# bdaiinstitute/judo

Hardware: AMD Instinct MI355X
Metric: rollouts/sec + plan-step ms, leap_cube MPPI 65536xH64 (higher is better)
Workload: dtype f32

## Files before the change

### include/judo_amd.h

```cpp
#ifndef JUDO_AMD_H
#define JUDO_AMD_H

#include <stddef.h>
#include <stdint.h>

#ifdef __cplusplus
extern "C" {
#endif

typedef struct jh_model jh_model;

enum jh_status {
  JH_OK = 0,
  JH_ERR_INVALID = -1,
  JH_ERR_HIP = -2,
  JH_ERR_UNSUPPORTED = -3,
  JH_ERR_BLOB = -4
};

enum jh_task_kind { JH_TASK_CARTPOLE = 0, JH_TASK_CYLINDER_PUSH = 1, JH_TASK_LEAP_CUBE = 2, JH_TASK_FR3_PICK = 3 };
enum jh_spline_kind { JH_SPLINE_ZERO = 0, JH_SPLINE_LINEAR = 1, JH_SPLINE_CUBIC = 3 };

#define JH_MAX_TASK_PARAMS 32
#define JH_MAX_KNOT_DIM 512
#define JH_MAX_ELITES 32

const char* jh_last_error(void);
int jh_version(void);

int jh_model_create(const void* blob, size_t nbytes, int device, jh_model** out);
void jh_model_destroy(jh_model* m);
int jh_model_dims(const jh_model* m, int* dims );

int jh_model_stats(jh_model* m, int* out , int reset);


int jh_model_set_self_collision(jh_model* m, int on);

int jh_model_set_contact_capacity(jh_model* m, int contacts);

int jh_model_build(const jh_model* m, int* out );

int jh_model_trace_layout(const jh_model* m, int* out );
int jh_trace_gather(const float* rec_in , int k, int stride_in, int n_offset, int n_local, const float* trace , int row_floats,
                    int colmajor, float* rec_out , void* stream);

int jh_model_limits(const jh_model* m, int* out );
int jh_model_max_fused_knots(const jh_model* m, int H);
int jh_model_one_launch_max_knots(const jh_model* m, int H);
int jh_model_set_plan_step_launches(jh_model* m, int launches);

int jh_upload_async(void* dst_device, const void* src_host, size_t nbytes, void* stream);
int jh_download_wait(void* dst_host, const void* src_device, size_t nbytes, void* stream);
int jh_download_begin(void* dst_host, const void* src_device, size_t nbytes, void* stream);
int jh_download_end(void);

int jh_rollout_cost(const jh_model* m, const float* x0, const float* nominal, const float* noise, int ldn, const float* sigma,
                    const float* W, const float* ctrl_lo_hi, const float* task_params, int phase, int N, int n_offset, int H, int K,
                    float* costs, float* knots_out, void* stream);
int jh_rollout_cost_traced(const jh_model* m, const float* x0, const float* nominal, const float* noise, int ldn, const float* sigma,
                    const float* W, const float* ctrl_lo_hi, const float* task_params, int phase, int N, int n_offset, int H, int K,
                    float* costs, float* knots_out, float* trace , void* stream);

int jh_rollout_materialize(const jh_model* m, const float* x0, int x0_batched, const float* controls, int N, int H, float* states,
                           float* sensors, void* stream);

int jh_task_reward(const jh_model* m, const float* states, const float* sensors, const float* controls, const float* task_params,
                   int phase, int N, int H, float* rewards, void* stream);

int jh_noise_normal(unsigned long long seed, unsigned int draw, int rows, int n_offset, int n_local, float* out, int ldn, void* stream);

int jh_sample_knots(const float* nominal, const float* noise, int ldn, const float* sigma, const float* ctrl_lo_hi ,
                    int N, int n_offset, int K, int nu, float* knots_nku, void* stream);

int jh_spline_controls(const float* W, const float* knots_nku, const float* nominal, const float* noise, int ldn, const float* sigma,
                       const float* ctrl_lo_hi, int N, int n_offset, int H, int K, int nu, float* controls, void* stream);

int jh_knot_moments(const float* knots_nku, const float* nominal, const float* noise, int ldn, const float* sigma, const float* ctrl_lo_hi,
                    const float* center, int N, int n_offset, int K, int nu, float* out, void* stream);

size_t jh_update_scratch_floats(int N, int K, int nu);
int jh_mppi_partial(const float* costs, const float* knots_nku, const float* nominal, const float* noise, int ldn, const float* sigma,
                    const float* ctrl_lo_hi, int N, int n_offset, int K, int nu, float lambda, float* scratch, float* rec, void* stream);
// ... 56 lines not shown
```

### judo_amd/_lib.py

```python

from __future__ import annotations

import ctypes as C
import os

_HERE = os.path.dirname(os.path.abspath(__file__))
LIB_PATH = os.environ.get("JUDO_AMD_LIB") or os.path.join(_HERE, "libjudo_amd.so")

_lib: C.CDLL | None = None

f32p = C.c_void_p

_SIGNATURES = {
    "jh_last_error": (C.c_char_p, []),
    "jh_version": (C.c_int, []),
    "jh_model_create": (C.c_int, [C.c_void_p, C.c_size_t, C.c_int, C.POINTER(C.c_void_p)]),
    "jh_model_destroy": (None, [C.c_void_p]),
    "jh_model_dims": (C.c_int, [C.c_void_p, C.POINTER(C.c_int)]),
    "jh_model_stats": (C.c_int, [C.c_void_p, C.POINTER(C.c_int), C.c_int]),
    "jh_model_set_kernel": (C.c_int, [C.c_void_p, C.c_int]),
    "jh_model_limits": (C.c_int, [C.c_void_p, C.POINTER(C.c_int)]),
    "jh_register_xcheck": (C.c_int, [C.c_void_p]),
    "jh_model_max_fused_knots": (C.c_int, [C.c_void_p, C.c_int]),
    "jh_model_one_launch_max_knots": (C.c_int, [C.c_void_p, C.c_int]),
    "jh_model_set_plan_step_launches": (C.c_int, [C.c_void_p, C.c_int]),
    "jh_model_set_self_collision": (C.c_int, [C.c_void_p, C.c_int]),
    "jh_model_set_contact_capacity": (C.c_int, [C.c_void_p, C.c_int]),
    "jh_model_build": (C.c_int, [C.c_void_p, C.POINTER(C.c_int)]),
    "jh_model_trace_layout": (C.c_int, [C.c_void_p, C.POINTER(C.c_int)]),
    "jh_trace_gather": (C.c_int, [C.c_void_p, C.c_int, C.c_int, C.c_int, C.c_int, C.c_void_p, C.c_int, C.c_int, C.c_void_p, C.c_void_p]),
    "jh_upload_async": (C.c_int, [C.c_void_p, C.c_void_p, C.c_size_t, C.c_void_p]),
    "jh_download_wait": (C.c_int, [C.c_void_p, C.c_void_p, C.c_size_t, C.c_void_p]),
    "jh_download_begin": (C.c_int, [C.c_void_p, C.c_void_p, C.c_size_t, C.c_void_p]),
    "jh_download_end": (C.c_int, []),
    "jh_rollout_cost": (C.c_int, [C.c_void_p, f32p, f32p, f32p, C.c_int, f32p, f32p, f32p, f32p, C.c_int, C.c_int, C.c_int, C.c_int, C.c_int, f32p, f32p, C.c_void_p]),
    "jh_rollout_cost_traced": (C.c_int, [C.c_void_p, f32p, f32p, f32p, C.c_int, f32p, f32p, f32p, f32p, C.c_int, C.c_int, C.c_int, C.c_int, C.c_int, f32p, f32p, f32p, C.c_void_p]),
    "jh_rollout_materialize": (C.c_int, [C.c_void_p, f32p, C.c_int, f32p, C.c_int, C.c_int, f32p, f32p, C.c_void_p]),
    "jh_task_reward": (C.c_int, [C.c_void_p, f32p, f32p, f32p, f32p, C.c_int, C.c_int, C.c_int, f32p, C.c_void_p]),
    "jh_noise_normal": (C.c_int, [C.c_ulonglong, C.c_uint, C.c_int, C.c_int, C.c_int, f32p, C.c_int, C.c_void_p]),
    "jh_sample_knots": (C.c_int, [f32p, f32p, C.c_int, f32p, f32p, C.c_int, C.c_int, C.c_int, C.c_int, f32p, C.c_void_p]),
    "jh_spline_controls": (C.c_int, [f32p, f32p, f32p, f32p, C.c_int, f32p, f32p, C.c_int, C.c_int, C.c_int, C.c_int, C.c_int, f32p, C.c_void_p]),
    "jh_knot_moments": (C.c_int, [f32p, f32p, f32p, C.c_int, f32p, f32p, f32p, C.c_int, C.c_int, C.c_int, C.c_int, f32p, C.c_void_p]),
    "jh_policy_create": (C.c_int, [C.POINTER(C.c_void_p), C.POINTER(C.c_void_p), C.POINTER(C.c_void_p)]),
    "jh_policy_destroy": (None, [C.c_void_p]),
    "jh_policy_scratch_floats": (C.c_size_t, [C.c_int]),
    "jh_policy_step": (C.c_int, [C.c_void_p, f32p, C.c_int, C.c_int, C.c_int, C.c_int, C.c_int, C.c_int, f32p, f32p, f32p, f32p, C.c_int, C.c_void_p]),
    "jh_tree_create": (C.c_int, [C.c_void_p, C.c_size_t, C.POINTER(C.c_void_p)]),
    "jh_tree_destroy": (None, [C.c_void_p]),
    "jh_tree_stats": (C.c_int, [C.c_void_p, C.POINTER(C.c_int), C.c_int]),
    "jh_tree_dims": (C.c_int, [C.c_void_p, C.POINTER(C.c_int)]),
    "jh_tree_set_self_collision": (C.c_int, [C.c_void_p, C.c_int]),
    "jh_tree_substeps": (C.c_int, [C.c_void_p, f32p, f32p, f32p, C.c_int, C.c_int, f32p, f32p, C.c_void_p]),
    "jh_policy_rollout_scratch_floats": (C.c_size_t, [C.c_int]),
    "jh_policy_rollout": (C.c_int, [C.c_void_p, C.c_void_p, f32p, C.c_int, f32p, f32p, f32p, C.c_int, C.c_int, C.c_int, C.c_int, C.c_double, f32p, f32p, f32p, C.POINTER(C.c_int), C.c_void_p]),
    "jh_update_scratch_floats": (C.c_size_t, [C.c_int, C.c_int, C.c_int]),
    "jh_mppi_partial": (C.c_int, [f32p, f32p, f32p, f32p, C.c_int, f32p, f32p, C.c_int, C.c_int, C.c_int, C.c_int, C.c_float, f32p, f32p, C.c_void_p]),
    "jh_mppi_merge": (C.c_int, [f32p, C.c_int, C.c_int, C.c_int, C.c_float, f32p, C.c_void_p]),
    "jh_topk_partial": (C.c_int, [f32p, f32p, f32p, f32p, C.c_int, f32p, f32p, C.c_int, C.c_int, C.c_int, C.c_int, C.c_int, C.c_int, f32p, f32p, C.c_void_p]),
# ... 62 lines not shown
```

### judo_amd/csrc/jh_api.hip

```cpp
#include <cmath>
#include <cstdlib>
#include <cstring>

#include "jh_internal.h"
#include "jh_update_dev.h"

static thread_local char g_err[512] = "";

void jh_set_error(const char* fmt, ...) {
  va_list ap;
  va_start(ap, fmt);
  vsnprintf(g_err, sizeof(g_err), fmt, ap);
  va_end(ap);
}

extern "C" const char* jh_last_error(void) { return g_err; }
extern "C" int jh_version(void) { return 100; }

static int image_cylinders(const jh_blob_header& h, const float* F, const int* I) {
  constexpr int HEADER = 24, BODY_I = 6, BODY_F = 32, BLOCK_I = 4, DOF_F = 20, ACT_I = 2, ACT_F = 8, GEOM_I = 2, GEOM_F = 20, GF_RBOUND = 15;
  if (h.nint < (uint32_t)HEADER || h.nfloat < (uint32_t)HEADER) return 0;
  const long NM = I[0], NBLK = I[1], nv = I[2], nu = I[4], NG = I[5];
  if (NM < 0 || NBLK < 0 || nv < 0 || nu < 0 || NG < 0) return 0;
  const long oI = HEADER + NM * BODY_I + NBLK * BLOCK_I + nu * ACT_I, oF = HEADER + NM * BODY_F + nv * DOF_F + nu * ACT_F;
// ... 5 lines not shown
    const float r = f[0], L = f[1], rb = f[GF_RBOUND], want = sqrtf(r * r + L * L);
    if (!(r > 0.f) || !(L > 0.f) || f[2] != 0.f) { jh_set_error("model_create: cylinder geom %ld: sizes must be (radius > 0, half length > 0, 0), got (%g, %g, %g)", g, r, L, f[2]); return -1; }
    if (!(fabsf(rb - want) <= 1e-5f * want)) { jh_set_error("model_create: cylinder geom %ld: bounding radius %g is not sqrt(r^2 + L^2) = %g", g, rb, want); return -1; }
    n++;
  }
  return n;
}

extern "C" int jh_model_create(const void* blob, size_t nbytes, int device, jh_model** out) {
  JH_REQUIRE(blob && out, "model_create: null pointer");
  if (nbytes < sizeof(jh_blob_header)) { jh_set_error("model_create: blob too small (%zu bytes)", nbytes); return JH_ERR_BLOB; }
  jh_blob_header h;
  memcpy(&h, blob, sizeof(h));
  if (h.magic != JH_BLOB_MAGIC || h.version != JH_BLOB_VERSION) { jh_set_error("model_create: bad magic/version (%08x, %u)", h.magic, h.version); return JH_ERR_BLOB; }
  size_t need = sizeof(h) + 4 * ((size_t)h.nfloat + h.nint);
  if (nbytes != need) { jh_set_error("model_create: blob size %zu != expected %zu", nbytes, need); return JH_ERR_BLOB; }
  if (h.kind > JH_TASK_FR3_PICK) { jh_set_error("model_create: unknown task kind %u", h.kind); return JH_ERR_BLOB; }
  if (h.kind == JH_TASK_CARTPOLE && h.nfloat < CP_NPARAM) { jh_set_error("model_create: cartpole blob has %u floats, need %d", h.nfloat, CP_NPARAM); return JH_ERR_BLOB; }
  if (h.kind == JH_TASK_CYLINDER_PUSH && h.nfloat < CY_NPARAM) { jh_set_error("model_create: cylinder blob has %u floats, need %d", h.nfloat, CY_NPARAM); return JH_ERR_BLOB; }
  if (h.ntaskparam > JH_MAX_TASK_PARAMS) { jh_set_error("model_create: too many task params"); return JH_ERR_BLOB; }
  int cylinders = 0;
  if (h.kind == JH_TASK_LEAP_CUBE || h.kind == JH_TASK_FR3_PICK) {
    const char* q = (const char*)blob + sizeof(h);
    std::vector<float> F((const float*)q, (const float*)q + h.nfloat);
    std::vector<int> I((const int*)(q + 4 * (size_t)h.nfloat), (const int*)(q + 4 * (size_t)h.nfloat) + h.nint);
    cylinders = image_cylinders(h, F.data(), I.data());
    if (cylinders < 0) return JH_ERR_BLOB;
    if (cylinders > 0 && h.kind != JH_TASK_LEAP_CUBE) { jh_set_error("model_create: %d cylinder geoms, and only the leap kernel has a cylinder build", cylinders); return JH_ERR_BLOB; }
  }
  JH_HIP(hipSetDevice(device));
  jh_model* m = new jh_model();
  m->device = device; m->kind = (int)h.kind; m->nq = h.nq; m->nv = h.nv; m->nu = h.nu; m->ns = h.ns; m->ntaskparam = h.ntaskparam;
  m->nf = h.nfloat; m->ni = h.nint; m->d_f = nullptr; m->d_i = nullptr; m->d_stats = nullptr; m->kernel_gen = (h.kind == JH_TASK_LEAP_CUBE || h.kind == JH_TASK_FR3_PICK) ? 3 : 2; m->self_collision = 1; m->contact_capacity = cylinders > 0 ? 64 : 48; m->cylinders = cylinders;
  { const char* e = getenv("JUDO_AMD_PLAN_STEP_LAUNCHES"); m->plan_step_launches = (e && e[0] == '2') ? 2 : 0; }
  const char* p = (const char*)blob + sizeof(h);
  m->h_f.assign((const float*)p, (const float*)p + h.nfloat);
  m->h_i.assign((const int*)(p + 4 * (size_t)h.nfloat), (const int*)(p + 4 * (size_t)h.nfloat) + h.nint);
  {
    hipMemPool_t pool = nullptr; int dev = 0;
    if (hipGetDevice(&dev) == hipSuccess && hipDeviceGetDefaultMemPool(&pool, dev) == hipSuccess && pool) {
      unsigned long long keep = ~0ull;
      (void)hipMemPoolSetAttribute(pool, hipMemPoolAttrReleaseThreshold, &keep);
    }
  }
  hipError_t e = hipMalloc(&m->d_f, 4 * (m->nf ? m->nf : 1));
  if (e == hipSuccess) e = hipMalloc(&m->d_i, 4 * (m->ni ? m->ni : 1));
  if (e == hipSuccess) e = hipMalloc(&m->d_stats, JH_NSTATS * sizeof(int));
  if (e == hipSuccess) e = hipMemset(m->d_stats, 0, JH_NSTATS * sizeof(int));
  if (e == hipSuccess && m->nf) e = hipMemcpy(m->d_f, m->h_f.data(), 4 * m->nf, hipMemcpyHostToDevice);
  if (e == hipSuccess && m->ni) e = hipMemcpy(m->d_i, m->h_i.data(), 4 * m->ni, hipMemcpyHostToDevice);
  if (e != hipSuccess) {
    jh_set_error("model_create: device upload failed: %s", hipGetErrorString(e));
    if (m->d_f) (void)hipFree(m->d_f);
    if (m->d_i) (void)hipFree(m->d_i);
    if (m->d_stats) (void)hipFree(m->d_stats);
    delete m;
    return JH_ERR_HIP;
  }
  *out = m;
  return JH_OK;
}

extern "C" void jh_model_destroy(jh_model* m) {
  if (!m) return;
  if (m->d_f) (void)hipFree(m->d_f);
  if (m->d_i) (void)hipFree(m->d_i);
// ... 104 lines not shown
static int max_fused_knots(const jh_model* m, int H) {
  const bool coop = m->kernel_gen >= 2 && (m->kind == JH_TASK_LEAP_CUBE || m->kind == JH_TASK_FR3_PICK);
  int k = JH_MAX_KNOT_DIM / (m->nu > 0 ? m->nu : 1);
  if (coop && m->kind == JH_TASK_LEAP_CUBE && m->kernel_gen >= 3) return k;
  if (coop) return k < 8 ? k : 8;
  const int lds_k = (m->kind == JH_TASK_CARTPOLE || m->kind == JH_TASK_CYLINDER_PUSH) ? jh_simple_max_knots(m, H) : (g_xcheck.max_knots ? g_xcheck.max_knots(m, H) : 0);
  return k < lds_k ? k : lds_k;
}

extern "C" int jh_model_limits(const jh_model* m, int* out) {
  JH_REQUIRE(m && out, "model_limits: null pointer");
  out[0] = max_fused_knots(m, 1);
  out[1] = JH_MAX_KNOT_DIM;
  out[2] = JH_MAX_ELITES;
  out[3] = m->kind == JH_TASK_LEAP_CUBE ? (m->kernel_gen >= 3 ? m->contact_capacity : 32) : (m->kind == JH_TASK_FR3_PICK ? (m->kernel_gen >= 3 ? 96 : 32) : 0);
  return JH_OK;
}

extern "C" int jh_model_max_fused_knots(const jh_model* m, int H) {
  JH_REQUIRE(m != nullptr && H >= 1, "model_max_fused_knots: null model or H < 1");
  return max_fused_knots(m, H);
}

extern "C" int jh_model_one_launch_max_knots(const jh_model* m, int H) {
  JH_REQUIRE(m != nullptr && H >= 1, "model_one_launch_max_knots: null model or H < 1");
  const int k = JH_MAX_KNOT_DIM / (m->nu > 0 ? m->nu : 1), lds_k = jh_simple_one_launch_max_knots(m, H);
  return k < lds_k ? k : lds_k;
}

extern "C" int jh_model_set_plan_step_launches(jh_model* m, int launches) {
  JH_REQUIRE(m != nullptr && launches >= 0 && launches <= 2, "model_set_plan_step_launches: launches must be 0 (automatic), 1 or 2");
  JH_REQUIRE(launches != 1 || m->kind == JH_TASK_CARTPOLE || m->kind == JH_TASK_CYLINDER_PUSH, "model_set_plan_step_launches: only the closed-form models have a one-launch plan step");
  m->plan_step_launches = launches;
  return JH_OK;
}

extern "C" int jh_upload_async(void* dst, const void* src, size_t nbytes, void* stream) {
  JH_REQUIRE(dst && src, "upload_async: null pointer");
  JH_HIP(hipMemcpyAsync(dst, src, nbytes, hipMemcpyHostToDevice, (hipStream_t)stream));
  return JH_OK;
}

extern "C" int jh_download_wait(void* dst, const void* src, size_t nbytes, void* stream) {
  JH_REQUIRE(dst && src, "download_wait: null pointer");
  JH_HIP(hipMemcpyAsync(dst, src, nbytes, hipMemcpyDeviceToHost, (hipStream_t)stream));
  JH_HIP(hipStreamSynchronize((hipStream_t)stream));
  return JH_OK;
}

namespace {
struct DlMark { void* stream; hipEvent_t ev; };
thread_local std::vector<DlMark> g_dl_marks;
struct DlPending { hipEvent_t ev; const unsigned* flag; unsigned expect; };
thread_local std::vector<DlPending> g_dl_pending;
}

static int download_begin(void* dst, const void* src, size_t nbytes, void* stream, const unsigned* flag, unsigned expect) {
  JH_REQUIRE(dst && src, "download_begin: null pointer");
  hipEvent_t ev = nullptr;
  for (const DlMark& mk : g_dl_marks) if (mk.stream == stream) ev = mk.ev;
  if (!ev) {
    int cur = 0, dev = 0;
    JH_HIP(hipGetDevice(&cur));
    dev = cur;
    if (stream) { hipDevice_t sd; if (hipStreamGetDevice((hipStream_t)stream, &sd) == hipSuccess) dev = (int)sd; else (void)hipGetLastError(); }
    if (dev != cur) JH_HIP(hipSetDevice(dev));
// ... 174 lines not shown
```

### judo_amd/csrc/jh_engine_v5.hip

```cpp
#include <cstddef>
#include <type_traits>

#include "jh_coop.h"

using namespace jh_eng;
using namespace jh_coop;

namespace {

constexpr int G = 16, RPW = 4, WAVE = 64;
constexpr int NCH = 4, NLK = 4;
#ifndef JH_V5_LSMAX
#define JH_V5_LSMAX 16
#endif
#ifndef JH_V5_LSKINK
#define JH_V5_LSKINK 0
#endif
#ifndef JH_V5_LSSHRINK
#define JH_V5_LSSHRINK 0.9f
#endif
#ifndef JH_V5_LSREV
#define JH_V5_LSREV 0.03f
#endif
#ifndef JH_V5_HCSPLIT
#define JH_V5_HCSPLIT 1
#endif
#ifndef JH_V5_C3CACHE
#define JH_V5_C3CACHE 1
#endif
#ifndef JH_V5_WORLDROT
#define JH_V5_WORLDROT 1
#endif
#ifndef JH_V5_HCMERGE
#define JH_V5_HCMERGE 1
#endif
#ifndef JH_V5_C3PAD
#define JH_V5_C3PAD 278
#endif
#ifndef JH_V5_LSRCP
#define JH_V5_LSRCP 1
#endif
// ... 355 lines not shown
}

__device__ __forceinline__ int pidx(int a, int b) { return a * (7 - a) / 2 + (b - a - 1); }
__device__ __forceinline__ bool chain_elim_order(int cmask, int c, int& level, int& parent, int& maxlev) {
  int adj[NCH] = {0, 0, 0, 0};
#pragma unroll
  for (int a = 0; a < NCH; a++)
#pragma unroll
    for (int b = a + 1; b < NCH; b++) if ((cmask >> (4 * a + b)) & 1) { adj[a] |= 1 << b; adj[b] |= 1 << a; }
  int rem = 0xF; bool ok = true;
  level = 0; parent = -1; maxlev = 0;
#pragma unroll
  for (int st = 0; st < NCH; st++) {
    int elig = 0, pr[NCH] = {-1, -1, -1, -1};
#pragma unroll
    for (int a = 0; a < NCH; a++) if ((rem >> a) & 1) {
      const int nbm = adj[a] & rem, deg = __popc(nbm);
      if (deg == 0) elig |= 1 << a;
      else if (deg == 1) {
        const int nb = __ffs(nbm) - 1;
        const int anb = nb == 0 ? adj[0] : (nb == 1 ? adj[1] : (nb == 2 ? adj[2] : adj[3]));
        if (__popc(anb & rem) > 1 || a < nb) { elig |= 1 << a; pr[a] = nb; }
      }
    }
    if (rem != 0 && elig == 0) ok = false;
    if (elig != 0) maxlev = st;
#pragma unroll
    for (int a = 0; a < NCH; a++) if (((elig >> a) & 1) && a == c) { level = st; parent = pr[a]; }
    rem &= ~elig;
  }
  return ok;
}

template <bool MATERIALIZE, int WPB, bool SELF>
#ifdef JH_V5_NUM_VGPR
#define JH_V5_REGATTR __attribute__((amdgpu_num_vgpr(JH_V5_NUM_VGPR)))
#else
#define JH_V5_REGATTR
#endif
__global__ __launch_bounds__(WAVE * WPB, JH_V5_WAVES_PER_EU) JH_V5_REGATTR void k_leap_v5(const float* __restrict__ gF, const int* __restrict__ gI, const float* __restrict__ x0, int x0_batched,
                                                   const float* __restrict__ nominal, const float* __restrict__ noise, int ldn,
                                                   const float* __restrict__ sigma, const float* __restrict__ W, const float* __restrict__ lohi,
                                                   const float* __restrict__ tp, int N, int n_offset, int H, int K, float* __restrict__ costs,
                                                   float* __restrict__ knots_out, const float* __restrict__ controls, float* __restrict__ states,
                                                   float* __restrict__ sensors, int* __restrict__ stats, int dshift, float* __restrict__ trace, float* __restrict__ ovf_all) {
#ifdef JH_V5_X_DYNRS
  extern __shared__ __attribute__((aligned(16))) unsigned char dynRS[];
  RS* sRS = reinterpret_cast<RS*>(dynRS);
#else
  __shared__ RS sRS[RPW * WPB];
#endif
  __shared__ float sBody[16 * JH_V5_BFS];
  __shared__ float sTp[16];
  __shared__ float sGeomF[MAXG * GEOM_F];
  __shared__ int sGeomI[MAXG * GEOM_I];
  __shared__ int sLaneG[16 * MAXLG];
  __shared__ float sLane[16 * LC_N];
  __shared__ int sBP[SELF ? 2 * MAXBP : 4];
  __shared__ int sBG[SELF ? 2 * NBC : 4];
  __shared__ float sBB[SELF ? NBC * 8 : 4];
#if JH_V5_KNOTS_LDS
  __shared__ float sKnAll[MAXK * WAVE * WPB];
#endif
  const int tid = threadIdx.x, wv = tid >> 6, lane = tid & 63, r = lane >> 4;
  int l = lane & 15, c = l >> 2, s = l & 3;
  RS& S = sRS[wv * RPW + r];
#if JH_V5_KNOTS_LDS
  float* sKn = sKnAll + wv * (MAXK * WAVE);
#endif
  const int nmI = gI[0], nblkI = gI[1], nuI = gI[4], ngI = gI[5], nsiteI = gI[6], nsI = gI[7], oRef = gI[18];
  const int oBodyF = HEADER_F, oDofF = oBodyF + nmI * BODY_F, oActF = oDofF + gI[2] * DOF_F, oGeomF = oActF + nuI * ACT_F, oSiteF = oGeomF + ngI * GEOM_F;
  const int oGeomI = HEADER_I + nmI * BODY_I + nblkI * BLOCK_I + nuI * ACT_I, oSiteI = oGeomI + ngI * GEOM_I;
  const int oLane = gI[11], lgm = gI[12];
  const int oBP = gI[15], oBS = gI[16], nBP = gI[17], oBG = oBP + 2 * nBP;
  for (int i = tid; i < 16 * BODY_F; i += WAVE * WPB) sBody[(i / BODY_F) * JH_V5_BFS + i % BODY_F] = gF[oBodyF + BODY_F + i];
  for (int i = tid; i < ngI * GEOM_F; i += WAVE * WPB) sGeomF[i] = gF[oGeomF + i];
  for (int i = tid; i < ngI * GEOM_I; i += WAVE * WPB) sGeomI[i] = gI[oGeomI + i];
  for (int i = tid; i < 16 * lgm; i += WAVE * WPB) sLaneG[i] = gI[oLane + i];
  if (!MATERIALIZE && tid < 9) sTp[tid] = tp[tid];
  if constexpr (SELF) {
    for (int i = tid; i < 2 * nBP && i < 2 * MAXBP; i += WAVE * WPB) sBP[i] = gI[oBP + i];
    for (int i = tid; i < 2 * NBC; i += WAVE * WPB) sBG[i] = gI[oBG + i];
    for (int i = tid; i < NBC * 8; i += WAVE * WPB) sBB[i] = gF[oBS + i];
  }
  if (tid < 16) {
    const float* df = gF + oDofF + (6 + l) * DOF_F; const float* af = gF + oActF + l * ACT_F;
    float* lc = sLane + l * LC_N;
    lc[LC_DAMP] = df[DF_DAMP]; lc[LC_KVD] = df[DF_KV]; lc[LC_FL] = df[DF_FL]; lc[LC_FB] = df[DF_FB]; lc[LC_FD] = df[DF_FD]; lc[LC_INVW] = df[DF_INVW];
    lc[LC_LIMITED] = df[DF_LIMITED]; lc[LC_LO] = df[DF_LO]; lc[LC_HI] = df[DF_HI]; lc[LC_LK] = df[DF_LK]; lc[LC_LB] = df[DF_LB];
    for (int k = 0; k < 5; k++) lc[LC_SI + k] = df[DF_SOLIMP + k];
    lc[LC_KP] = af[AF_KP]; lc[LC_KV] = af[AF_KV]; lc[LC_CLIM] = af[AF_CLIM]; lc[LC_CLO] = af[AF_CLO]; lc[LC_CHI] = af[AF_CHI];
    lc[LC_IMCK] = l < 6 ? 1.f / (l < 3 ? gF[HF_CMASS] : gF[HF_CINERTIA + (l < 3 ? 0 : l - 3)]) : 0.f;
  }
  const float* lc = sLane + l * LC_N;
  const int n = ((blockIdx.x * WPB + wv) << (2 - dshift)) + (r >> dshift);
  const bool live = n < N && (r & ((1 << dshift) - 1)) == 0;
  const int nc = n < N ? n : N - 1;
  const float h = gF[HF_DT], impratio = gF[HF_IMPRATIO], tol = gF[HF_TOL], lstol = gF[HF_LSTOL]; const int cap = (int)gF[HF_MAXITER];
  const float grav[3] = {gF[HF_GRAV], gF[HF_GRAV + 1], gF[HF_GRAV + 2]};
  const float cmass = gF[HF_CMASS], cI[3] = {gF[HF_CINERTIA], gF[HF_CINERTIA + 1], gF[HF_CINERTIA + 2]};
  const float chs[3] = {gF[HF_CSIZE], gF[HF_CSIZE + 1], gF[HF_CSIZE + 2]}, crb = gF[HF_CRBOUND], ctran = gF[HF_CTRAN];
  const float cK = gF[HF_CK], cB = gF[HF_CB];
  float csi[5]; for (int k = 0; k < 5; k++) csi[k] = gF[HF_SOLIMP + k];
  const float mck = (l < 3 ? cmass : (l == 3 ? cI[0] : (l == 4 ? cI[1] : (l == 5 ? cI[2] : 0.f))));
  float q, qd, qc[7], vc[6];
  {
    const float* xi = x0 + ((MATERIALIZE && x0_batched) ? (size_t)nc * NX : 0);
    for (int k = 0; k < 7; k++) qc[k] = xi[k];
    for (int k = 0; k < 6; k++) vc[k] = xi[NQ + k];
    q = xi[7 + l]; qd = xi[NQ + 6 + l];
  }
  auto knot_at = [&](int k, int ll, int ncc) -> float {
    const int i = k * NU + ll;
    float v = nominal[i];
    if (n_offset + ncc != 0) v = fmaf(sigma[i], noise[(size_t)i * ldn + ncc], v);
    return jh_clampf(v, lohi[ll], lohi[NU + ll]);
  };
  if (!MATERIALIZE) {
#if JH_V5_KNOTS_LDS
    for (int k = 0; k < MAXK; k++) sKn[k * WAVE + lane] = k < K ? knot_at(k, l, nc) : 0.f;
#endif
    if (knots_out && live) for (int k = 0; k < K; k++) knots_out[(size_t)(k * NU + l) * ldn + n] = knot_at(k, l, nc);
  }
  S.ws[6 + l] = 0.f; if (l < 6) S.ws[l] = 0.f;
  if (l < 4) S.cmd[l] = l == 0 ? cmass : (l == 1 ? cI[0] : (l == 2 ? cI[1] : cI[2]));
  int n_iters = 0, n_maxed = 0, n_wave_iters = 0;
  float acc = 0.f;
#ifdef JH_V5_TICKS
  long long cyc[16] = {0, 0, 0, 0, 0, 0, 0, 0, 0, 0, 0, 0, 0, 0, 0, 0}, t0 = clock64();
#define V5_TICK(slot) { long long t__ = clock64(); cyc[slot] += t__ - t0; t0 = t__; }
#else
#define V5_TICK(slot)
#endif
#ifdef JH_V5_COUNT
  int cnt_dense = 0, cnt_it = 0, cnt_l2 = 0, cnt_bp = 0, cnt_hh = 0, cnt_cls[4] = {0, 0, 0, 0};
#endif
  __syncthreads();

  for (int hh = 0; hh < H; hh++) {
#if JH_V5_OPAQUE_LANE
    OPAQUE(l); c = l >> 2; s = l & 3;
    const float* lc = sLane + l * LC_N;
#endif
    float u;
    if (MATERIALIZE) u = controls[((size_t)nc * H + hh) * NU + l];
    else {
      u = 0.f;
#if JH_V5_KNOTS_LDS
      for (int k = 0; k < K && k < MAXK; k++) u = fmaf(W[hh * K + k], sKn[k * WAVE + lane], u);
#else
      {
        int lo_ = lane; OPAQUE(lo_);
        const int n_ = ((blockIdx.x * WPB + wv) << (2 - dshift)) + ((lo_ >> 4) >> dshift), nc_ = n_ < N ? n_ : N - 1;
        for (int k = 0; k < K; k++) u = fmaf(W[hh * K + k], knot_at(k, l, nc_), u);
      }
#endif
    }
    float Mrow[NLK], fs_own, a0_own;
    {
      float ax[NLK][3], og[NLK][3], Rown[9], pown[3];
      {
        float nn = rsqrtf(qc[3] * qc[3] + qc[4] * qc[4] + qc[5] * qc[5] + qc[6] * qc[6]);
        qc[3] *= nn; qc[4] *= nn; qc[5] *= nn; qc[6] *= nn;
        float Rc[9]; quat2mat(Rc, qc + 3);
        float P[3] = {0, 0, 0}, R[9] = {1, 0, 0, 0, 1, 0, 0, 0, 1};
        float sn_own, cs_own; sincosf(q, &sn_own, &cs_own);
#pragma unroll
        for (int j = 0; j < NLK; j++) {
          const float* bf = sBody + (4 * c + j) * JH_V5_BFS;
          float P2[3], R0[9];
          if (j == 0) { for (int k = 0; k < 3; k++) P2[k] = bf[BF_LPOS + k]; for (int k = 0; k < 9; k++) R0[k] = bf[BF_LR + k]; }
          else { mulMV(P2, R, bf + BF_LPOS); for (int k = 0; k < 3; k++) P2[k] += P[k]; mulMM(R0, R, bf + BF_LR); }
          const float* al = bf + BF_AXIS;
          mulMV(ax[j], R0, al);
          for (int k = 0; k < 3; k++) { og[j][k] = P2[k]; P[k] = P2[k]; }
          const float sn = quad_get(sn_own, j), cs = quad_get(cs_own, j), t = 1.f - cs, x = al[0], y = al[1], z = al[2];
          float Rq[9] = {t * x * x + cs, t * x * y - sn * z, t * x * z + sn * y, t * x * y + sn * z, t * y * y + cs, t * y * z - sn * x, t * x * z - sn * y, t * y * z + sn * x, t * z * z + cs};
          mulMM(R, R0, Rq);
          if (j == s) { for (int k = 0; k < 3; k++) pown[k] = P2[k]; for (int k = 0; k < 9; k++) Rown[k] = R[k]; }
        }
        for (int k = 0; k < 3; k++) { S.pa[1 + l][k] = pown[k]; S.pa[1 + l][4 + k] = s == 0 ? ax[0][k] : (s == 1 ? ax[1][k] : (s == 2 ? ax[2][k] : ax[3][k])); }
        for (int k = 0; k < 9; k++) S.xR[1 + l][k] = Rown[k];
        if (l == 0) { for (int k = 0; k < 3; k++) S.pa[0][k] = qc[k]; for (int k = 0; k < 9; k++) S.xR[0][k] = Rc[k]; S.ncon = 0; S.nhit = 0; }
        S.qv[6 + l] = qd;
        if (l < 6) S.qv[l] = vc[l];
      }
// ... 1143 lines not shown
      if (ang > 0.f) {
        float sn, cs; sincosf(0.5f * ang, &sn, &cs); float kk = sn / wn;
        float dq[4] = {cs, vc[3] * kk, vc[4] * kk, vc[5] * kk}, *qq = qc + 3;
        float r0 = qq[0] * dq[0] - qq[1] * dq[1] - qq[2] * dq[2] - qq[3] * dq[3];
        float r1 = qq[0] * dq[1] + qq[1] * dq[0] + qq[2] * dq[3] - qq[3] * dq[2];
        float r2 = qq[0] * dq[2] - qq[1] * dq[3] + qq[2] * dq[0] + qq[3] * dq[1];
        float r3 = qq[0] * dq[3] + qq[1] * dq[2] - qq[2] * dq[1] + qq[3] * dq[0];
        qq[0] = r0; qq[1] = r1; qq[2] = r2; qq[3] = r3;
      }
      float nn = rsqrtf(qc[3] * qc[3] + qc[4] * qc[4] + qc[5] * qc[5] + qc[6] * qc[6]);
      qc[3] *= nn; qc[4] *= nn; qc[5] *= nn; qc[6] *= nn;
    }
    V5_TICK(7)
    if (MATERIALIZE) {
      if (states && live) {
        float* o = states + ((size_t)nc * H + hh) * NX;
        o[7 + l] = q; o[NQ + 6 + l] = qd;
        if (l < 7) o[l] = qc[l];
        if (l < 6) o[NQ + l] = vc[l];
      }
    } else acc += leap_step_cost(sTp, qc);
    WSYNC();
  }
#ifdef JH_V5_COUNT
  if (stats) { if (lane == 0) { atomicAdd(stats + 24, cnt_dense); atomicAdd(stats + 25, cnt_it); atomicAdd(stats + 26, cnt_l2); atomicAdd(stats + 28, H); } if (l == 0 && live) { atomicAdd(stats + 27, cnt_bp); atomicAdd(stats + 29, cnt_hh); for (int k = 0; k < 4; k++) atomicAdd(stats + 30 + k, cnt_cls[k]); } }
#endif
#ifdef JH_V5_TICKS
  if (lane == 0 && stats) { for (int k = 0; k < 8; k++) atomicAdd((unsigned long long*)(stats + 4) + k, (unsigned long long)cyc[k]);
                            for (int k = 0; k < 16; k++) atomicAdd((unsigned long long*)(stats + 384) + k, (unsigned long long)cyc[k]); }
#endif
  if (!MATERIALIZE && live && l == 0) costs[n] = acc / (float)H;
  if (stats && live && l == 0) { if (n_maxed) atomicAdd(stats + 1, n_maxed); atomicAdd(stats + 2, n_iters); atomicAdd(stats + 3, H); }
  if (stats && lane == 0 && live) { atomicAdd(stats + 20, n_wave_iters); atomicAdd(stats + 21, H); }
}

bool model_is_leap(const jh_model* m) {
  return m->kind == JH_TASK_LEAP_CUBE && m->nq == 23 && m->nv == 22 && m->nu == 16 && (m->ns == NS || (m->ns == NS_CALTECH && m->h_i.size() > 18 && m->h_i[18] > 0)) && m->h_i.size() > 17 &&
         m->h_i[0] == 17 && m->h_i[1] == 4 && m->h_i[11] > 0 && m->h_i[5] <= MAXG && m->h_i[12] <= MAXLG && m->h_i[17] <= MAXBP
#if JH_V5_WORLDROT
         && m->h_f.size() > (size_t)HF_CINERTIA + 2 && m->h_f[HF_CINERTIA] == m->h_f[HF_CINERTIA + 1] && m->h_f[HF_CINERTIA] == m->h_f[HF_CINERTIA + 2]
#endif
         ;
}

}

#ifdef JH_V5_X_DYNRS
#define JH_V5_DYNBYTES (sizeof(RS) * RPW * JH_V5_WPB)
#else
#define JH_V5_DYNBYTES 0
#endif
#ifndef JH_V5_NAME
#define JH_V5_NAME(f) f
#endif
int JH_V5_NAME(jh_engine5_rollout_cost)(const jh_model* m, const float* x0, const float* nominal, const float* noise, int ldn, const float* sigma, const float* W,
                            const float* lohi, const float* tp, int N, int n_offset, int H, int K, float* costs, float* knots_out, float* trace, hipStream_t st) {
  if (!model_is_leap(m)) { jh_set_error("rollout_cost: the cooperative engine kernel is instantiated for leap_cube only"); return JH_ERR_UNSUPPORTED; }
  if ((m->cylinders > 0) != (JH_V5_CYL != 0)) { jh_set_error("rollout_cost: an image with cylinder geoms runs on the cylinder build of the leap kernel and no other image does (%d cylinders)", m->cylinders); return JH_ERR_UNSUPPORTED; }
#if JH_V5_KNOTS_LDS
  JH_REQUIRE(K <= MAXK, "rollout_cost: the cooperative leap kernel keeps at most 8 knots per actuator (K=%d)", K);
#endif
  const int dshift = jh_latency_shift(N, RPW); const int per_block = (RPW >> dshift) * JH_V5_WPB;
  int grid = (N + per_block - 1) / per_block;
  float* ovf = nullptr;
  if (NOVF > 0) ovf = jh_launch_scratch(m, (size_t)N * NOVF * POOL_F * sizeof(float), st);
  if (m->self_collision && m->h_i[17] > 0)
    hipLaunchKernelGGL((k_leap_v5<false, JH_V5_WPB, true>), dim3(grid), dim3(WAVE * JH_V5_WPB), JH_V5_DYNBYTES, st, m->d_f, m->d_i, x0, 0, nominal, noise, ldn, sigma, W, lohi, tp, N, n_offset, H, K, costs,
                       knots_out, (const float*)nullptr, (float*)nullptr, (float*)nullptr, m->d_stats, dshift, trace, ovf);
  else
    hipLaunchKernelGGL((k_leap_v5<false, JH_V5_WPB, false>), dim3(grid), dim3(WAVE * JH_V5_WPB), JH_V5_DYNBYTES, st, m->d_f, m->d_i, x0, 0, nominal, noise, ldn, sigma, W, lohi, tp, N, n_offset, H, K, costs,
                       knots_out, (const float*)nullptr, (float*)nullptr, (float*)nullptr, m->d_stats, dshift, trace, ovf);
  return jh_launch_done(ovf, st);
}

int JH_V5_NAME(jh_engine5_materialize)(const jh_model* m, const float* x0, int x0_batched, const float* controls, int N, int H, float* states, float* sensors,
                           hipStream_t st) {
  if (!model_is_leap(m)) { jh_set_error("rollout_materialize: the cooperative engine kernel is instantiated for leap_cube only"); return JH_ERR_UNSUPPORTED; }
  if ((m->cylinders > 0) != (JH_V5_CYL != 0)) { jh_set_error("rollout_materialize: an image with cylinder geoms runs on the cylinder build of the leap kernel and no other image does (%d cylinders)", m->cylinders); return JH_ERR_UNSUPPORTED; }
  const int dshift = jh_latency_shift(N, RPW); const int per_block = (RPW >> dshift) * JH_V5_WPB;
  int grid = (N + per_block - 1) / per_block;
  float* ovf = nullptr;
  if (NOVF > 0) ovf = jh_launch_scratch(m, (size_t)N * NOVF * POOL_F * sizeof(float), st);
  if (m->self_collision && m->h_i[17] > 0)
    hipLaunchKernelGGL((k_leap_v5<true, JH_V5_WPB, true>), dim3(grid), dim3(WAVE * JH_V5_WPB), JH_V5_DYNBYTES, st, m->d_f, m->d_i, x0, x0_batched, (const float*)nullptr, (const float*)nullptr, 0,
                       (const float*)nullptr, (const float*)nullptr, (const float*)nullptr, (const float*)nullptr, N, 0, H, 0, (float*)nullptr, (float*)nullptr,
                       controls, states, sensors, m->d_stats, dshift, (float*)nullptr, ovf);
  else
    hipLaunchKernelGGL((k_leap_v5<true, JH_V5_WPB, false>), dim3(grid), dim3(WAVE * JH_V5_WPB), JH_V5_DYNBYTES, st, m->d_f, m->d_i, x0, x0_batched, (const float*)nullptr, (const float*)nullptr, 0,
                       (const float*)nullptr, (const float*)nullptr, (const float*)nullptr, (const float*)nullptr, N, 0, H, 0, (float*)nullptr, (float*)nullptr,
                       controls, states, sensors, m->d_stats, dshift, (float*)nullptr, ovf);
  return jh_launch_done(ovf, st);
}
```

### judo_amd/csrc/jh_internal.h

```cpp
#pragma once

#include <hip/hip_runtime.h>

#include <cstdarg>
#include <cstdint>
#include <cstdio>
#include <vector>

#include "judo_amd.h"
#include "judo_amd_xcheck.h"

#define JH_BLOB_MAGIC 0x314D484Au
#define JH_BLOB_VERSION 1u
#define JH_NSTATS 512

struct jh_blob_header {
  uint32_t magic, version, kind, nq, nv, nu, ns, ntaskparam, nfloat, nint;
  uint32_t reserved[6];
};

struct jh_model {
  int device, kind, nq, nv, nu, ns, ntaskparam;
  size_t nf, ni;
  float* d_f;
  int* d_i;
  int kernel_gen;
  int contact_capacity;
  int cylinders;
  int self_collision;
  int plan_step_launches;
  mutable int one_launch_steps = 0;
  mutable int ovf_fallbacks = 0;
  int* d_stats;
  std::vector<float> h_f;
  std::vector<int> h_i;
};

void jh_set_error(const char* fmt, ...);

inline float* jh_launch_scratch(const jh_model* m, size_t bytes, hipStream_t st) {
  hipMemPool_t pool = nullptr; void* p = nullptr;
  if (hipDeviceGetDefaultMemPool(&pool, m->device) == hipSuccess && pool && hipMallocFromPoolAsync(&p, bytes, pool, st) == hipSuccess) return (float*)p;
  (void)hipGetLastError();
  if (__atomic_fetch_add(&m->ovf_fallbacks, 1, __ATOMIC_RELAXED) == 0)
    fprintf(stderr, "judo_amd: no stream-ordered scratch for the contacts above the LDS pool (%zu bytes): this launch runs with the LDS capacity alone; see jh_model_stats out[6]\n", bytes);
  return nullptr;
}

#define JH_HIP(call)                                                                      \
  do {                                                                                    \
    hipError_t e__ = (call);                                                              \
    if (e__ != hipSuccess) {                                                              \
      jh_set_error("%s failed: %s (%s:%d)", #call, hipGetErrorString(e__), __FILE__, __LINE__); \
      return JH_ERR_HIP;                                                                  \
    }                                                                                     \
  } while (0)

inline int jh_launch_done(float* ovf, hipStream_t st) {
  const hipError_t e = hipGetLastError();
  const hipError_t f = ovf ? hipFreeAsync(ovf, st) : hipSuccess;
  if (e != hipSuccess) { jh_set_error("kernel launch failed: %s", hipGetErrorString(e)); return JH_ERR_HIP; }
  if (f != hipSuccess) { jh_set_error("hipFreeAsync failed: %s", hipGetErrorString(f)); return JH_ERR_HIP; }
  return JH_OK;
}

#define JH_REQUIRE(cond, ...)    \
  do {                           \
    if (!(cond)) {               \
      jh_set_error(__VA_ARGS__); \
      return JH_ERR_INVALID;     \
    }                            \
  } while (0)

enum {
  CP_DT = 0, CP_G, CP_MCART, CP_MPOLE, CP_L, CP_IPOLE, CP_DAMP_X, CP_DAMP_TH, CP_KP, CP_KV, CP_CTRL_LO, CP_CTRL_HI, CP_CTRL_LIMITED,
  CP_FRC_LO, CP_FRC_HI, CP_FRC_LIMITED, CP_X_LO, CP_X_HI, CP_X_LIMITED, CP_LIM_K, CP_LIM_B, CP_SOLIMP0, CP_SOLIMP1, CP_SOLIMP2,
// ... 75 lines not shown
```

### judo_amd/device.py

```python

from __future__ import annotations

import ctypes as C
import os

import numpy as np
import torch

from judo_amd import _lib
from judo_amd.models import layout, load_description, pack_model


def require_gpu() -> torch.device:
    if not torch.cuda.is_available():
        raise RuntimeError("judo_amd needs an MI355X (HIP device): torch.cuda.is_available() is False and there is no CPU fallback")
    return torch.device("cuda", torch.cuda.current_device())


_raw_stream = getattr(torch._C, "_cuda_getCurrentRawStream", None)


def current_stream_ptr() -> int:
    if _raw_stream is not None:
        return int(_raw_stream(torch.cuda.current_device()))
# ... 86 lines not shown
        _lib.check(_lib.lib().jh_model_trace_layout(self.handle, out), "jh_model_trace_layout")
        return int(out[0]), int(out[1]), bool(out[2])

    def limits(self) -> tuple[int, int, int, int]:
        out = (C.c_int * 4)()
        _lib.check(_lib.lib().jh_model_limits(self.handle, out), "jh_model_limits")
        return tuple(int(v) for v in out)

    @property
    def max_fused_knots(self) -> int:
        out = (C.c_int * 4)()
        _lib.check(_lib.lib().jh_model_limits(self.handle, out), "jh_model_limits")
        return int(out[0])

    def max_fused_knots_at(self, H: int) -> int:
        H = int(H)
        k = self._max_knots_cache.get(H)
        if k is None:
            k = int(_lib.lib().jh_model_max_fused_knots(self.handle, H))
            if k < 0:
                _lib.check(k, "jh_model_max_fused_knots")
            self._max_knots_cache[H] = k
        return k

    def one_launch_max_knots_at(self, H: int) -> int:
        k = int(_lib.lib().jh_model_one_launch_max_knots(self.handle, int(H)))
        if k < 0:
            _lib.check(k, "jh_model_one_launch_max_knots")
        return k

    def set_plan_step_launches(self, launches: int) -> None:
        _lib.check(_lib.lib().jh_model_set_plan_step_launches(self.handle, int(launches)), "jh_model_set_plan_step_launches")

    def stats(self, reset: bool = True) -> dict:
        out = (C.c_int * 8)()
        _lib.check(_lib.lib().jh_model_stats(self.handle, out, int(reset)), "jh_model_stats")
        u = [v & 0xFFFFFFFF for v in out]
        return {"contact_overflow": u[0], "newton_cap_hits": u[1], "newton_iters": u[2], "steps": u[3], "wave_newton_iters": u[4], "wave_steps": u[5], "overflow_pool_fallbacks": u[6], "one_launch_plan_steps": u[7]}

    def __del__(self) -> None:
        try:
            if getattr(self, "handle", None):
                _lib.lib().jh_model_destroy(self.handle)
                self.handle = None
        except Exception:
            pass
```

Measured before the change: 1.126 million.

## Add persistent-wave work-stealing schedule for leap_cube rollout cost kernel

Adds a persistent-kernel mode to the v5 leap rollout kernel. The grid is capped at two blocks per CU, and each wave pulls further rollout groups from a global atomic counter until all are done. The aim is to balance the uneven per-rollout cost from contact and Newton iteration counts, avoiding tail waves left idle under a static grid. It is on by default when the grid exceeds the slot count and dshift is 0, and it costs an atomic per group, a memset, and a scratch allocation.

```diff
diff --git a/include/judo_amd.h b/include/judo_amd.h
--- a/include/judo_amd.h
+++ b/include/judo_amd.h
@@ -49,6 +49,7 @@
 int jh_model_max_fused_knots(const jh_model* m, int H);
 int jh_model_one_launch_max_knots(const jh_model* m, int H);
 int jh_model_set_plan_step_launches(jh_model* m, int launches);
+int jh_model_set_rollout_schedule(jh_model* m, int mode);
 
 int jh_upload_async(void* dst_device, const void* src_host, size_t nbytes, void* stream);
 int jh_download_wait(void* dst_host, const void* src_device, size_t nbytes, void* stream);
diff --git a/judo_amd/_lib.py b/judo_amd/_lib.py
--- a/judo_amd/_lib.py
+++ b/judo_amd/_lib.py
@@ -24,6 +24,7 @@
     "jh_model_max_fused_knots": (C.c_int, [C.c_void_p, C.c_int]),
     "jh_model_one_launch_max_knots": (C.c_int, [C.c_void_p, C.c_int]),
     "jh_model_set_plan_step_launches": (C.c_int, [C.c_void_p, C.c_int]),
+    "jh_model_set_rollout_schedule": (C.c_int, [C.c_void_p, C.c_int]),
     "jh_model_set_self_collision": (C.c_int, [C.c_void_p, C.c_int]),
     "jh_model_set_contact_capacity": (C.c_int, [C.c_void_p, C.c_int]),
     "jh_model_build": (C.c_int, [C.c_void_p, C.POINTER(C.c_int)]),
diff --git a/judo_amd/csrc/jh_api.hip b/judo_amd/csrc/jh_api.hip
--- a/judo_amd/csrc/jh_api.hip
+++ b/judo_amd/csrc/jh_api.hip
@@ -61,6 +61,7 @@
   jh_model* m = new jh_model();
   m->device = device; m->kind = (int)h.kind; m->nq = h.nq; m->nv = h.nv; m->nu = h.nu; m->ns = h.ns; m->ntaskparam = h.ntaskparam;
   m->nf = h.nfloat; m->ni = h.nint; m->d_f = nullptr; m->d_i = nullptr; m->d_stats = nullptr; m->kernel_gen = (h.kind == JH_TASK_LEAP_CUBE || h.kind == JH_TASK_FR3_PICK) ? 3 : 2; m->self_collision = 1; m->contact_capacity = cylinders > 0 ? 64 : 48; m->cylinders = cylinders;
+  { const char* e = getenv("JUDO_AMD_ROLLOUT_SCHEDULE"); m->rollout_schedule = (e && (e[0] == '1' || e[0] == '2')) ? e[0] - '0' : 0; }
   { const char* e = getenv("JUDO_AMD_PLAN_STEP_LAUNCHES"); m->plan_step_launches = (e && e[0] == '2') ? 2 : 0; }
   const char* p = (const char*)blob + sizeof(h);
   m->h_f.assign((const float*)p, (const float*)p + h.nfloat);
@@ -231,6 +232,12 @@
   JH_REQUIRE(m != nullptr && launches >= 0 && launches <= 2, "model_set_plan_step_launches: launches must be 0 (automatic), 1 or 2");
   JH_REQUIRE(launches != 1 || m->kind == JH_TASK_CARTPOLE || m->kind == JH_TASK_CYLINDER_PUSH, "model_set_plan_step_launches: only the closed-form models have a one-launch plan step");
   m->plan_step_launches = launches;
+  return JH_OK;
+}
+
+extern "C" int jh_model_set_rollout_schedule(jh_model* m, int mode) {
+  JH_REQUIRE(m != nullptr && mode >= 0 && mode <= 2, "model_set_rollout_schedule: mode must be 0 (automatic), 1 (static grid) or 2 (persistent waves wherever the kernel has them)");
+  m->rollout_schedule = mode;
   return JH_OK;
 }
 
diff --git a/judo_amd/csrc/jh_engine_v5.hip b/judo_amd/csrc/jh_engine_v5.hip
--- a/judo_amd/csrc/jh_engine_v5.hip
+++ b/judo_amd/csrc/jh_engine_v5.hip
@@ -7,6 +7,11 @@
 using namespace jh_coop;
 
 namespace {
+
+#ifdef JH_V5_WAVESTAMP
+__device__ unsigned long long* g_wavestamp = nullptr;
+__device__ int g_wavestamp_cap = 0;
+#endif
 
 constexpr int G = 16, RPW = 4, WAVE = 64;
 constexpr int NCH = 4, NLK = 4;
@@ -428,7 +433,7 @@
   return ok;
 }
 
-template <bool MATERIALIZE, int WPB, bool SELF>
+template <bool MATERIALIZE, int WPB, bool SELF, bool PERSIST = false>
 #ifdef JH_V5_NUM_VGPR
 #define JH_V5_REGATTR __attribute__((amdgpu_num_vgpr(JH_V5_NUM_VGPR)))
 #else
@@ -439,7 +444,7 @@
                                                    const float* __restrict__ sigma, const float* __restrict__ W, const float* __restrict__ lohi,
                                                    const float* __restrict__ tp, int N, int n_offset, int H, int K, float* __restrict__ costs,
                                                    float* __restrict__ knots_out, const float* __restrict__ controls, float* __restrict__ states,
-                                                   float* __restrict__ sensors, int* __restrict__ stats, int dshift, float* __restrict__ trace, float* __restrict__ ovf_all) {
+                                                   float* __restrict__ sensors, int* __restrict__ stats, int dshift_, float* __restrict__ trace, float* __restrict__ ovf_all, unsigned* __restrict__ head) {
 #ifdef JH_V5_X_DYNRS
   extern __shared__ __attribute__((aligned(16))) unsigned char dynRS[];
   RS* sRS = reinterpret_cast<RS*>(dynRS);
@@ -457,6 +462,11 @@
   __shared__ float sBB[SELF ? NBC * 8 : 4];
 #if JH_V5_KNOTS_LDS
   __shared__ float sKnAll[MAXK * WAVE * WPB];
+#endif
+  __shared__ int sGrp[WPB];
+  const int dshift = PERSIST ? 0 : dshift_;
+#ifdef JH_V5_WAVESTAMP
+  const unsigned long long ws_entry = wall_clock64(); unsigned long long ws_staged = ws_entry;
 #endif
   const int tid = threadIdx.x, wv = tid >> 6, lane = tid & 63, r = lane >> 4;
   int l = lane & 15, c = l >> 2, s = l & 3;
@@ -489,7 +499,20 @@
     lc[LC_IMCK] = l < 6 ? 1.f / (l < 3 ? gF[HF_CMASS] : gF[HF_CINERTIA + (l < 3 ? 0 : l - 3)]) : 0.f;
   }
   const float* lc = sLane + l * LC_N;
-  const int n = ((blockIdx.x * WPB + wv) << (2 - dshift)) + (r >> dshift);
+  int grp = blockIdx.x * WPB + wv;
+  const int ngroups = (N + RPW - 1) / RPW;
+  if constexpr (PERSIST) {
+    __syncthreads();
+#ifdef JH_V5_WAVESTAMP
+    ws_staged = wall_clock64();
+#endif
+  }
+  for (; !PERSIST || grp < ngroups;) {
+  if constexpr (PERSIST) { if (lane == 0) sGrp[wv] = grp; }
+#ifdef JH_V5_WAVESTAMP
+  const unsigned long long ws_start = wall_clock64();
+#endif
+  const int n = (grp << (2 - dshift)) + (r >> dshift);
   const bool live = n < N && (r & ((1 << dshift) - 1)) == 0;
   const int nc = n < N ? n : N - 1;
   const float h = gF[HF_DT], impratio = gF[HF_IMPRATIO], tol = gF[HF_TOL], lstol = gF[HF_LSTOL]; const int cap = (int)gF[HF_MAXITER];
@@ -531,7 +554,13 @@
 #ifdef JH_V5_COUNT
   int cnt_dense = 0, cnt_it = 0, cnt_l2 = 0, cnt_bp = 0, cnt_hh = 0, cnt_cls[4] = {0, 0, 0, 0};
 #endif
-  __syncthreads();
+  if constexpr (PERSIST) WSYNC();
+  else {
+    __syncthreads();
+#ifdef JH_V5_WAVESTAMP
+    ws_staged = wall_clock64();
+#endif
+  }
 
   for (int hh = 0; hh < H; hh++) {
 #if JH_V5_OPAQUE_LANE
@@ -547,7 +576,8 @@
 #else
       {
         int lo_ = lane; OPAQUE(lo_);
-        const int n_ = ((blockIdx.x * WPB + wv) << (2 - dshift)) + ((lo_ >> 4) >> dshift), nc_ = n_ < N ? n_ : N - 1;
+        const int g_ = PERSIST ? sGrp[wv] : (int)(blockIdx.x * WPB + wv);
+        const int n_ = (g_ << (2 - dshift)) + ((lo_ >> 4) >> dshift), nc_ = n_ < N ? n_ : N - 1;
         for (int k = 0; k < K; k++) u = fmaf(W[hh * K + k], knot_at(k, l, nc_), u);
       }
 #endif
@@ -1757,6 +1787,19 @@
   if (!MATERIALIZE && live && l == 0) costs[n] = acc / (float)H;
   if (stats && live && l == 0) { if (n_maxed) atomicAdd(stats + 1, n_maxed); atomicAdd(stats + 2, n_iters); atomicAdd(stats + 3, H); }
   if (stats && lane == 0 && live) { atomicAdd(stats + 20, n_wave_iters); atomicAdd(stats + 21, H); }
+#ifdef JH_V5_WAVESTAMP
+  if (lane == 0 && g_wavestamp && grp < g_wavestamp_cap) {
+    unsigned long long* w = g_wavestamp + (size_t)grp * 6;
+    w[0] = ((unsigned long long)blockIdx.x << 32) | ((unsigned long long)wv << 8) | (__smid() & 0xff); w[1] = ws_entry; w[2] = ws_staged; w[3] = ws_start; w[4] = wall_clock64(); w[5] = 1;
+  }
+#endif
+  if constexpr (!PERSIST) break;
+  else {
+    int t = 0;
+    if (lane == 0) t = (int)atomicAdd(head, 1u);
+    grp = (int)(gridDim.x * WPB) + __builtin_amdgcn_readfirstlane(t);
+  }
+  }
 }
 
 bool model_is_leap(const jh_model* m) {
@@ -1768,6 +1811,11 @@
          ;
 }
 
+int device_cus(const jh_model* m) {
+  int v = 0;
+  return (hipDeviceGetAttribute(&v, hipDeviceAttributeMultiprocessorCount, m->device) == hipSuccess && v > 0) ? v : 256;
+}
+
 }
 
 #ifdef JH_V5_X_DYNRS
@@ -1777,6 +1825,13 @@
 #endif
 #ifndef JH_V5_NAME
 #define JH_V5_NAME(f) f
+#endif
+#ifdef JH_V5_WAVESTAMP
+extern "C" int JH_V5_NAME(jh_v5_wavestamp_buffer)(unsigned long long* buf, int groups) {
+  JH_HIP(hipMemcpyToSymbol(HIP_SYMBOL(g_wavestamp), &buf, sizeof(buf)));
+  JH_HIP(hipMemcpyToSymbol(HIP_SYMBOL(g_wavestamp_cap), &groups, sizeof(groups)));
+  return JH_OK;
+}
 #endif
 int JH_V5_NAME(jh_engine5_rollout_cost)(const jh_model* m, const float* x0, const float* nominal, const float* noise, int ldn, const float* sigma, const float* W,
                             const float* lohi, const float* tp, int N, int n_offset, int H, int K, float* costs, float* knots_out, float* trace, hipStream_t st) {
@@ -1787,15 +1842,22 @@
 #endif
   const int dshift = jh_latency_shift(N, RPW); const int per_block = (RPW >> dshift) * JH_V5_WPB;
   int grid = (N + per_block - 1) / per_block;
-  float* ovf = nullptr;
-  if (NOVF > 0) ovf = jh_launch_scratch(m, (size_t)N * NOVF * POOL_F * sizeof(float), st);
-  if (m->self_collision && m->h_i[17] > 0)
-    hipLaunchKernelGGL((k_leap_v5<false, JH_V5_WPB, true>), dim3(grid), dim3(WAVE * JH_V5_WPB), JH_V5_DYNBYTES, st, m->d_f, m->d_i, x0, 0, nominal, noise, ldn, sigma, W, lohi, tp, N, n_offset, H, K, costs,
-                       knots_out, (const float*)nullptr, (float*)nullptr, (float*)nullptr, m->d_stats, dshift, trace, ovf);
-  else
-    hipLaunchKernelGGL((k_leap_v5<false, JH_V5_WPB, false>), dim3(grid), dim3(WAVE * JH_V5_WPB), JH_V5_DYNBYTES, st, m->d_f, m->d_i, x0, 0, nominal, noise, ldn, sigma, W, lohi, tp, N, n_offset, H, K, costs,
-                       knots_out, (const float*)nullptr, (float*)nullptr, (float*)nullptr, m->d_stats, dshift, trace, ovf);
-  return jh_launch_done(ovf, st);
+  bool persist = dshift == 0 && m->rollout_schedule != 1; int slots = 0;
+  if (persist) { slots = 2 * device_cus(m); persist = m->rollout_schedule == 2 || grid > slots; }
+  const size_t ovf_bytes = NOVF > 0 ? (size_t)N * NOVF * POOL_F * sizeof(float) : 0;
+  float* scratch = nullptr; float* ovf = nullptr; unsigned* head = nullptr;
+  if (ovf_bytes > 0 || persist) scratch = jh_launch_scratch(m, ovf_bytes + (persist ? 16 : 0), st, ovf_bytes > 0);
+  if (scratch && persist && hipMemsetAsync(scratch, 0, 16, st) != hipSuccess) { (void)hipGetLastError(); persist = false; }
+  if (!scratch) persist = false;
+  if (persist) { head = (unsigned*)scratch; if (grid > slots) grid = slots; }
+  if (scratch && ovf_bytes > 0) ovf = scratch + (head ? 4 : 0);
+#define JH_V5_LAUNCH_COST(SELF_, PERSIST_)                                                                                                                                        \
+  hipLaunchKernelGGL((k_leap_v5<false, JH_V5_WPB, SELF_, PERSIST_>), dim3(grid), dim3(WAVE * JH_V5_WPB), JH_V5_DYNBYTES, st, m->d_f, m->d_i, x0, 0, nominal, noise, ldn, sigma, W, \
+                     lohi, tp, N, n_offset, H, K, costs, knots_out, (const float*)nullptr, (float*)nullptr, (float*)nullptr, m->d_stats, dshift, trace, ovf, head)
+  if (m->self_collision && m->h_i[17] > 0) { if (persist) JH_V5_LAUNCH_COST(true, true); else JH_V5_LAUNCH_COST(true, false); }
+  else { if (persist) JH_V5_LAUNCH_COST(false, true); else JH_V5_LAUNCH_COST(false, false); }
+#undef JH_V5_LAUNCH_COST
+  return jh_launch_done(scratch, st);
 }
 
 int JH_V5_NAME(jh_engine5_materialize)(const jh_model* m, const float* x0, int x0_batched, const float* controls, int N, int H, float* states, float* sensors,
@@ -1809,10 +1871,10 @@
   if (m->self_collision && m->h_i[17] > 0)
     hipLaunchKernelGGL((k_leap_v5<true, JH_V5_WPB, true>), dim3(grid), dim3(WAVE * JH_V5_WPB), JH_V5_DYNBYTES, st, m->d_f, m->d_i, x0, x0_batched, (const float*)nullptr, (const float*)nullptr, 0,
                        (const float*)nullptr, (const float*)nullptr, (const float*)nullptr, (const float*)nullptr, N, 0, H, 0, (float*)nullptr, (float*)nullptr,
-                       controls, states, sensors, m->d_stats, dshift, (float*)nullptr, ovf);
+                       controls, states, sensors, m->d_stats, dshift, (float*)nullptr, ovf, (unsigned*)nullptr);
   else
     hipLaunchKernelGGL((k_leap_v5<true, JH_V5_WPB, false>), dim3(grid), dim3(WAVE * JH_V5_WPB), JH_V5_DYNBYTES, st, m->d_f, m->d_i, x0, x0_batched, (const float*)nullptr, (const float*)nullptr, 0,
                        (const float*)nullptr, (const float*)nullptr, (const float*)nullptr, (const float*)nullptr, N, 0, H, 0, (float*)nullptr, (float*)nullptr,
-                       controls, states, sensors, m->d_stats, dshift, (float*)nullptr, ovf);
+                       controls, states, sensors, m->d_stats, dshift, (float*)nullptr, ovf, (unsigned*)nullptr);
   return jh_launch_done(ovf, st);
 }
diff --git a/judo_amd/csrc/jh_internal.h b/judo_amd/csrc/jh_internal.h
--- a/judo_amd/csrc/jh_internal.h
+++ b/judo_amd/csrc/jh_internal.h
@@ -28,6 +28,7 @@
   int contact_capacity;
   int cylinders;
   int self_collision;
+  int rollout_schedule;
   int plan_step_launches;
   mutable int one_launch_steps = 0;
   mutable int ovf_fallbacks = 0;
@@ -38,10 +39,11 @@
 
 void jh_set_error(const char* fmt, ...);
 
-inline float* jh_launch_scratch(const jh_model* m, size_t bytes, hipStream_t st) {
+inline float* jh_launch_scratch(const jh_model* m, size_t bytes, hipStream_t st, bool overflow_rows = true) {
   hipMemPool_t pool = nullptr; void* p = nullptr;
   if (hipDeviceGetDefaultMemPool(&pool, m->device) == hipSuccess && pool && hipMallocFromPoolAsync(&p, bytes, pool, st) == hipSuccess) return (float*)p;
   (void)hipGetLastError();
+  if (!overflow_rows) return nullptr;
   if (__atomic_fetch_add(&m->ovf_fallbacks, 1, __ATOMIC_RELAXED) == 0)
     fprintf(stderr, "judo_amd: no stream-ordered scratch for the contacts above the LDS pool (%zu bytes): this launch runs with the LDS capacity alone; see jh_model_stats out[6]\n", bytes);
   return nullptr;
diff --git a/judo_amd/device.py b/judo_amd/device.py
--- a/judo_amd/device.py
+++ b/judo_amd/device.py
@@ -142,6 +142,9 @@
     def set_plan_step_launches(self, launches: int) -> None:
         _lib.check(_lib.lib().jh_model_set_plan_step_launches(self.handle, int(launches)), "jh_model_set_plan_step_launches")
 
+    def set_rollout_schedule(self, mode: int) -> None:
+        _lib.check(_lib.lib().jh_model_set_rollout_schedule(self.handle, int(mode)), "jh_model_set_rollout_schedule")
+
     def stats(self, reset: bool = True) -> dict:
         out = (C.c_int * 8)()
         _lib.check(_lib.lib().jh_model_stats(self.handle, out, int(reset)), "jh_model_stats")
```

New measurement: 1.196 million (median of 6 runs). 1.06x the previous value.
